# raphaelsulzer/dgnn

Measured on AMD Instinct MI355X. Metric: tetrahedra/sec (in/out classified), 1M-tet graph at 1/2/4/8 MI355X, higher is better.
Workload: dtype f32 (fp16x2-split products, 22-bit operands; `exact_f32` = bit-faithful fp32 products)

## Files before the change

### dgnn_amd/csrc/fused_ws.hip

```cpp
#include <stdlib.h>

#include "common.h"
#include "fused_common.h"

namespace {
using namespace fused;

typedef float f32x4_t __attribute__((ext_vector_type(4)));
#define H8(v) __builtin_bit_cast(f16x8, v)

constexpr int WS_C = 128;
constexpr int WS_TILE = 32;
constexpr int WS_NP = 8;
template <int CIN> struct WsC {
    static constexpr int NCH = CIN / 16;
    static constexpr int NV = NCH / 4;
    static constexpr int KH = CIN / 32;
    static constexpr int PP = CIN / 8;
    static constexpr int ROWB = 8 * CIN;
    static constexpr int SLOT = WS_TILE * ROWB;
    static constexpr int BP = NCH * 2 * 48 * 16;
};
template <int CIN, int RING> struct WsL {
    static constexpr int OFF_BP = RING * WsC<CIN>::SLOT;
    static constexpr int OFF_ROWF = OFF_BP + WsC<CIN>::BP;
    static constexpr int OFF_CST = OFF_ROWF + RING * WS_TILE * 4;
    static constexpr int OFF_SC = OFF_CST + 3 * WS_C * 4;
    static constexpr int OFF_DC = OFF_SC + 16 + 2 * RING * 4 + 16 + 16;
    static constexpr int OFF_PLOG = OFF_DC + (64 + 64 + 128 + 4) * 4;
    static constexpr int OFF_YS = OFF_PLOG + 2 * 4 * 32 * 8;
    static constexpr int OFF_CMAX = OFF_YS + 2 * 32 * 4;
    static constexpr int OFF_W0S = OFF_CMAX + 4 * 32 * 4;
    static constexpr int OFF_W0 = (OFF_W0S + 32 + 255) & ~255;
    static constexpr int OFF_YT = OFF_W0 + 4 * 4 * 2 * 64 * 16;
    static constexpr int SMEM = OFF_SC + 16 + 2 * RING * 4 + 16 + 16;
    static constexpr int SMEM_DEC = OFF_YT + 2 * 4 * 2 * 2 * 64 * 16;
    static_assert(SMEM_DEC <= 160 * 1024, "the LDS of one CU");
};

struct WsDec {
    const float* W0;
    const float* b0;
    const float* scale1;
    const float* shift1;
    const float* W3;
    const float* b3;
    float* logits;
};


__device__ __forceinline__ void st_nt16(float* p, f32x4_t v) { __builtin_nontemporal_store(v, reinterpret_cast<f32x4_t*>(p)); }
typedef uint32_t u32x2_t __attribute__((ext_vector_type(2)));
__device__ __forceinline__ float ub16_lo(uint32_t u) { return __builtin_fabsf(__builtin_bit_cast(float, u << 15)); }
__device__ __forceinline__ float ub16_hi(uint32_t u) { return __builtin_bit_cast(float, (u >> 16) << 15); }
__device__ __forceinline__ uint32_t ub16_enc(float v) {
    const uint32_t b = __builtin_bit_cast(uint32_t, v) & 0x7FFFFFFFu;
    return (b + 0x3FFFu + ((b >> 15) & 1u)) >> 15;
}
__device__ __forceinline__ uint32_t bits(float f) { return __builtin_bit_cast(uint32_t, f); }

constexpr int WS_KNOBS = 1 | (0 << 4);
template <int CIN, int RING, bool DEC, bool IO16 = false, bool LDC = false>
__global__ void __launch_bounds__(1024) k_sage_fused_ws(const int32_t* __restrict__ rowptr, const int32_t* __restrict__ src, const int32_t* __restrict__ eid,
                                                        int64_t n_dst, const float* __restrict__ x, const float* __restrict__ xdst, int64_t ldx_arg,
                                                        const float* __restrict__ ea, int64_t lde, const float* __restrict__ We, const float* __restrict__ be,
                                                        const float* __restrict__ Wj, const float* __restrict__ bj, const float* __restrict__ Wi,
                                                        const float* __restrict__ scale, const float* __restrict__ shift, int relu, float* __restrict__ out,
                                                        int64_t ldo, int64_t ntiles, int knobs, WsDec dec) {
    static_assert(CIN == 128 || (CIN == 64 && !DEC), "input widths of the shipped model's 128-wide layers");
    static_assert(!IO16 || !DEC, "the decoder-carrying launch of the bf16-storage chain stays with fused_bf16.hip");
    const int64_t ldx = LDC ? (int64_t)CIN : ldx_arg;
    const uint16_t* const x16 = reinterpret_cast<const uint16_t*>(x);
    const uint16_t* const xdst16 = reinterpret_cast<const uint16_t*>(xdst);
    uint16_t* const out16 = reinterpret_cast<uint16_t*>(out);
    typedef WsC<CIN> G;
    constexpr int NCH = G::NCH, NV = G::NV, KH = G::KH, PP = G::PP;
    extern __shared__ __attribute__((aligned(16))) char ws_smem[];
    const bool nt_store = (knobs & 1) != 0;
    typedef WsL<CIN, RING> L;
    char* const ring = ws_smem;
    char* const bpbuf = ws_smem + L::OFF_BP;
    float* const rowf = reinterpret_cast<float*>(ws_smem + L::OFF_ROWF);
    float* const cst = reinterpret_cast<float*>(ws_smem + L::OFF_CST);
    uint32_t* const scbuf = reinterpret_cast<uint32_t*>(ws_smem + L::OFF_SC);
    volatile uint32_t* const ready = reinterpret_cast<volatile uint32_t*>(ws_smem + L::OFF_SC + 16);
    volatile uint32_t* const done = ready + RING;
    volatile uint32_t* const ycnt = done + RING;
    volatile uint32_t* const yfree = ycnt + 2;
    volatile uint32_t* const lcnt = ycnt + 4;
    volatile uint32_t* const ccnt = ycnt + 6;
    float* const dcst = reinterpret_cast<float*>(ws_smem + L::OFF_DC);
    float* const plog = reinterpret_cast<float*>(ws_smem + L::OFF_PLOG);
    float* const ysc = reinterpret_cast<float*>(ws_smem + L::OFF_YS);
    uint32_t* const cmax = reinterpret_cast<uint32_t*>(ws_smem + L::OFF_CMAX);
    uint32_t* const w0max = reinterpret_cast<uint32_t*>(ws_smem + L::OFF_W0S);
    float* const w0inv = reinterpret_cast<float*>(ws_smem + L::OFF_W0S + 16);
    char* const w0buf = ws_smem + L::OFF_W0;
    char* const ytile = ws_smem + L::OFF_YT;
    typedef __attribute__((address_space(3))) volatile uint32_t lds_vu32;
    auto wait_for = [&](volatile uint32_t* ctr, uint32_t target) {
        asm volatile("" ::: "memory");
        lds_vu32* c3 = (lds_vu32*)ctr;
        while ((int32_t)(__builtin_amdgcn_readfirstlane((int)*c3) - (int)target) < 0) __builtin_amdgcn_s_sleep(1);
        asm volatile("" ::: "memory");
    };
    const int lane = lane_id(), w = wave_id_uniform();
    const int jcol = lane & 15, tq = lane >> 4;

    const int nwg = gridDim.x, xcd = blockIdx.x & 7, slot_ = blockIdx.x >> 3, wg_per_xcd = (nwg + 7 - xcd) >> 3;
    const int64_t per = (ntiles + 7) / 8, t_lo = xcd * per, t_hi = min(ntiles, t_lo + per);
    int64_t my_n = 0;
    if (t_lo + slot_ < t_hi) my_n = (t_hi - t_lo - slot_ + wg_per_xcd - 1) / wg_per_xcd;
    auto tile_of = [&](int64_t it) { return t_lo + slot_ + it * wg_per_xcd; };

    if (threadIdx.x == 0) scbuf[0] = 0u;
    if (threadIdx.x < 2 * RING + 8) ready[threadIdx.x] = 0u;
    if constexpr (DEC) {
        for (int n_ = threadIdx.x; n_ < 64; n_ += blockDim.x) {
            const float s1 = dec.scale1 ? dec.scale1[n_] : 1.f, h1 = dec.scale1 ? dec.shift1[n_] : 0.f;
            dcst[n_] = s1;
            dcst[64 + n_] = __fmaf_rn(dec.b0[n_], s1, h1);
            dcst[128 + n_] = dec.W3[n_];
            dcst[192 + n_] = dec.W3[64 + n_];
        }
        if (threadIdx.x < 2) dcst[256 + threadIdx.x] = dec.b3[threadIdx.x];
        if (threadIdx.x < 4 * WS_TILE) cmax[threadIdx.x] = 0u;
        if (threadIdx.x < 4) w0max[threadIdx.x] = 0u;
    }
    __syncthreads();
    if constexpr (DEC) {
#pragma unroll
        for (int hb = 0; hb < 4; ++hb) {
            uint32_t m0 = 0u;
            for (int e = threadIdx.x; e < 16 * WS_C; e += blockDim.x) m0 = umax(m0, absbits(dec.W0[hb * 16 * WS_C + e]));
            m0 = wave_umax(m0);
            if ((threadIdx.x & 63) == 0) atomicMax(&w0max[hb], m0);
        }
    }
    {
        uint32_t me = 0u;
        for (int e = threadIdx.x; e < CIN * FE; e += blockDim.x) me = umax(me, absbits(We[e]));
        for (int e = threadIdx.x; e < CIN; e += blockDim.x) me = umax(me, absbits(be[e]));
        me = wave_umax(me);
        if (lane == 0) atomicMax(&scbuf[0], me);
    }
    for (int c = threadIdx.x; c < WS_C; c += blockDim.x) {
        cst[c] = bj ? bj[c] : 0.f;
        cst[WS_C + c] = scale ? scale[c] : 1.f;
        cst[2 * WS_C + c] = scale ? shift[c] : 0.f;
    }
    __syncthreads();
    float sWe, inv_sWe;
    pow2_scales(scbuf[0], sWe, inv_sWe);
    constexpr bool LINE_OWN = !IO16 && NV == 2;
    auto chan = [](int j, int cb) { return LINE_OWN ? ((cb >> 2) * 64 + 4 * j + (cb & 3)) : NCH * j + cb; };
    for (int e = threadIdx.x; e < NCH * 48; e += blockDim.x) {
        const int cb = e / 48, gj = e - cb * 48, g = gj >> 4, j = gj & 15;
        const int c = chan(j, cb);
        uint32_t ph[4], pl[4];
#pragma unroll
        for (int d = 0; d < 4; ++d) {
            float v[2];
#pragma unroll
            for (int u = 0; u < 2; ++u) {
                const int k = 8 * g + 2 * d + u;
                v[u] = k < FE ? We[(int64_t)c * FE + k] : (k == FE ? be[c] : 0.f);
            }
            split2h(v[0] * sWe, v[1] * sWe, ph[d], pl[d]);
        }
        uint4* dst = reinterpret_cast<uint4*>(bpbuf + ((cb * 2) * 48 + gj) * 16);
        dst[0] = make_uint4(ph[0], ph[1], ph[2], ph[3]);
        dst[48] = make_uint4(pl[0], pl[1], pl[2], pl[3]);
    }

    auto stage_b = [&](uint32_t t, int hb, int b) {
        wait_for(ycnt + (t & 1), 8u * (t / 2 + 1));
        int ln = lane;
        asm volatile("" : "+v"(ln));
        const char* yt = ytile + ((t & 1) << 14) + ((b * 128 + ln) << 4);
        const char* wp = w0buf + ((hb * 512 + ln) << 4);
        const float inv = ysc[(t & 1) * WS_TILE + 16 * b + (ln & 15)] * w0inv[hb];
        f32x4_t hs = {0.f, 0.f, 0.f, 0.f};
#pragma unroll
        for (int s = 0; s < 4; ++s) {
            const f16x8 w0h = H8(*reinterpret_cast<const uint4*>(wp + (s << 11))), w0l = H8(*reinterpret_cast<const uint4*>(wp + (s << 11) + 1024));
            const f16x8 yh = H8(*reinterpret_cast<const uint4*>(yt + (s << 12))), yl = H8(*reinterpret_cast<const uint4*>(yt + (s << 12) + 1024));
            hs = __builtin_amdgcn_mfma_f32_16x16x32_f16(w0l, yh, hs, 0, 0, 0);
            hs = __builtin_amdgcn_mfma_f32_16x16x32_f16(w0h, yl, hs, 0, 0, 0);
            hs = __builtin_amdgcn_mfma_f32_16x16x32_f16(w0h, yh, hs, 0, 0, 0);
        }
        asm volatile("s_waitcnt lgkmcnt(0)" ::: "memory");
        if (lane == 0) atomicAdd(const_cast<uint32_t*>(yfree + (t & 1)), 1u);
#pragma unroll
        for (int i = 0; i < 4; ++i) hs[i] *= inv;
        const int u0 = 16 * hb + 4 * (ln >> 4);
        float l0 = 0.f, l1 = 0.f;
#pragma unroll
        for (int i = 0; i < 4; ++i) {
            const float hv = fmaxf(__fmaf_rn(hs[i], dcst[u0 + i], dcst[64 + u0 + i]), 0.f);
            l0 = __fmaf_rn(hv, dcst[128 + u0 + i], l0);
            l1 = __fmaf_rn(hv, dcst[192 + u0 + i], l1);
        }
        l0 = cross_row_sum(l0);
        l1 = cross_row_sum(l1);
        if (ln < 16) *reinterpret_cast<float2*>(plog + (((t & 1) * 4 + hb) * WS_TILE + 16 * b + ln) * 2) = make_float2(l0, l1);
        asm volatile("s_waitcnt lgkmcnt(0)" ::: "memory");
        if (lane == 0) atomicAdd(const_cast<uint32_t*>(lcnt + (t & 1)), 1u);
    };

    const int bsel = (knobs >> 4) & 3;
    auto b_on_consumers = [&](uint32_t t) { return bsel == 0 ? false : bsel == 1 ? (t & 1) == 0 : bsel == 2 ? (t & 3) != 3 : true; };

    if (w >= WS_NP) {
        const int cw = w - WS_NP;
        const int col = 16 * cw + jcol;
        uint32_t mw = 0u;
#pragma unroll
        for (int s = 0; s < 2 * KH; ++s) {
            const float* wr = (s < KH ? Wj : Wi) + (int64_t)col * CIN + 32 * (s % KH) + 8 * tq;
            const f32x4_t r0 = *reinterpret_cast<const f32x4_t*>(wr), r1 = *reinterpret_cast<const f32x4_t*>(wr + 4);
#pragma unroll
            for (int i = 0; i < 4; ++i) mw = umax(mw, umax(absbits(r0[i]), absbits(r1[i])));
        }
        float sW, inv_sW;
        pow2_scales(wave_umax(mw), sW, inv_sW);
        f16x8 wh[2 * KH], wl[2 * KH];
#pragma unroll
        for (int s = 0; s < 2 * KH; ++s) {
            const float* wr = (s < KH ? Wj : Wi) + (int64_t)col * CIN + 32 * (s % KH) + 8 * tq;
            const f32x4_t r0 = *reinterpret_cast<const f32x4_t*>(wr), r1 = *reinterpret_cast<const f32x4_t*>(wr + 4);
            uint32_t ph[4], pl[4];
            split2h(r0[0] * sW, r0[1] * sW, ph[0], pl[0]);
            split2h(r0[2] * sW, r0[3] * sW, ph[1], pl[1]);
            split2h(r1[0] * sW, r1[1] * sW, ph[2], pl[2]);
            split2h(r1[2] * sW, r1[3] * sW, ph[3], pl[3]);
            wh[s] = pack8h(ph);
            wl[s] = pack8h(pl);
        }
        if constexpr (DEC) {
#pragma unroll
            for (int u = 0; u < 2; ++u) {
                const int hb = 2 * (cw & 1) + u, ks = cw >> 1;
                float sW0, inv_sW0;
                pow2_scales(w0max[hb], sW0, inv_sW0);
                if (ks == 0 && lane == 0) w0inv[hb] = inv_sW0;
                const float* wr = dec.W0 + (int64_t)(16 * hb + jcol) * WS_C + 32 * ks + 8 * tq;
                const f32x4_t r0 = *reinterpret_cast<const f32x4_t*>(wr), r1 = *reinterpret_cast<const f32x4_t*>(wr + 4);
                uint32_t ph[4], pl[4];
                split2h(r0[0] * sW0, r0[1] * sW0, ph[0], pl[0]);
                split2h(r0[2] * sW0, r0[3] * sW0, ph[1], pl[1]);
                split2h(r1[0] * sW0, r1[1] * sW0, ph[2], pl[2]);
                split2h(r1[2] * sW0, r1[3] * sW0, ph[3], pl[3]);
                uint4* dst = reinterpret_cast<uint4*>(w0buf + (((hb * 4 + ks) * 128 + lane) << 4));
                dst[0] = make_uint4(ph[0], ph[1], ph[2], ph[3]);
                dst[64] = make_uint4(pl[0], pl[1], pl[2], pl[3]);
            }
        }
        __syncthreads();
        const int c0 = 16 * cw + 4 * tq;
        const int64_t n_it = my_n + (DEC ? 3 : 0);
        f32x4_t yp[2] = {{0.f, 0.f, 0.f, 0.f}, {0.f, 0.f, 0.f, 0.f}}, yn[2] = {yp[0], yp[1]};
        for (int64_t it = 1; it <= n_it; ++it) {
            if constexpr (DEC) {
                if (cw == 0 && it >= 4) {
                    const uint32_t t = (uint32_t)(it - 4);
                    wait_for(lcnt + (t & 1), 8u * (t / 2 + 1));
                    if (lane < WS_TILE) {
                        float s0 = dcst[256], s1 = dcst[257];
#pragma unroll
                        for (int q = 0; q < 4; ++q) {
                            const float* pq = plog + (((t & 1) * 4 + q) * WS_TILE + lane) * 2;
                            s0 += pq[0];
                            s1 += pq[1];
                        }
                        const int64_t cell = tile_of(t) * WS_TILE + lane;
                        if (cell < n_dst) *reinterpret_cast<float2*>(dec.logits + cell * 2) = make_float2(s0, s1);
                    }
                }
            }
            if (it >= 1 && it <= my_n) {
                const int sl = (int)((it - 1) % RING);
                wait_for(ready + sl, (uint32_t)(WS_NP * ((it - 1) / RING + 1)));
                f32x4_t acc[2] = {{0.f, 0.f, 0.f, 0.f}, {0.f, 0.f, 0.f, 0.f}};
                int key = jcol ^ tq;
                asm volatile("" : "+v"(key));
                uint32_t rbase[4];
#pragma unroll
                for (int m = 0; m < 4; ++m) {
                    rbase[m] = (uint32_t)(sl * G::SLOT + jcol * G::ROWB) + (uint32_t)(((4 * m) ^ key) << 4);
                    asm volatile("" : "+v"(rbase[m]));
                }
                f16x8 xh[2][2], xl[2][2];
                auto ld_step = [&](int s, int set) {
#pragma unroll
                    for (int b = 0; b < 2; ++b) {
                        const char* rp = ring + rbase[s & 3] + (16 * b * G::ROWB + ((s >> 2) << 8));
                        xh[set][b] = H8(*reinterpret_cast<const uint4*>(rp));
                        xl[set][b] = H8(*reinterpret_cast<const uint4*>(rp + 2 * PP * 16));
                    }
                };
                ld_step(0, 0);
#pragma unroll
                for (int s = 0; s < 2 * KH; ++s) {
                    const int set = s & 1;
                    if (s + 1 < 2 * KH) ld_step(s + 1, set ^ 1);
                    __builtin_amdgcn_sched_barrier(0);
#pragma unroll
                    for (int b = 0; b < 2; ++b) acc[b] = __builtin_amdgcn_mfma_f32_16x16x32_f16(wl[s], xh[set][b], acc[b], 0, 0, 0);
#pragma unroll
                    for (int b = 0; b < 2; ++b) acc[b] = __builtin_amdgcn_mfma_f32_16x16x32_f16(wh[s], xl[set][b], acc[b], 0, 0, 0);
#pragma unroll
                    for (int b = 0; b < 2; ++b) acc[b] = __builtin_amdgcn_mfma_f32_16x16x32_f16(wh[s], xh[set][b], acc[b], 0, 0, 0);
                    __builtin_amdgcn_sched_barrier(0);
                }
                float invr[2];
#pragma unroll
                for (int b = 0; b < 2; ++b) invr[b] = rowf[sl * WS_TILE + 16 * b + jcol] * inv_sW;
                asm volatile("s_waitcnt lgkmcnt(0)" ::: "memory");
                if (lane == 0) atomicAdd(const_cast<uint32_t*>(done + sl), 1u);
                const f32x4_t bb = *reinterpret_cast<const f32x4_t*>(cst + c0), sc = *reinterpret_cast<const f32x4_t*>(cst + WS_C + c0),
                              sh = *reinterpret_cast<const f32x4_t*>(cst + 2 * WS_C + c0);
                f32x4_t yv[2];
#pragma unroll
                for (int b = 0; b < 2; ++b) {
#pragma unroll
                    for (int i = 0; i < 4; ++i) {
                        float t_ = __fmaf_rn(acc[b][i], invr[b], bb[i]);
                        t_ = __fmaf_rn(t_, sc[i], sh[i]);
                        yv[b][i] = relu ? fmaxf(t_, 0.f) : t_;
                    }
                }
                if constexpr (!DEC) {
                    const int64_t cell0 = tile_of(it - 1) * WS_TILE;
#pragma unroll
                    for (int b = 0; b < 2; ++b) {
                        const int64_t cell = cell0 + 16 * b + jcol;
                        if (cell < n_dst) {
                            if constexpr (IO16) {
                                const u32x2_t pk = {ub16_enc(yv[b][0]) | (ub16_enc(yv[b][1]) << 16), ub16_enc(yv[b][2]) | (ub16_enc(yv[b][3]) << 16)};
                                if (nt_store) __builtin_nontemporal_store(pk, reinterpret_cast<u32x2_t*>(out16 + cell * ldo + c0));
                                else *reinterpret_cast<u32x2_t*>(out16 + cell * ldo + c0) = pk;
                            } else {
                                if (nt_store) st_nt16(out + cell * ldo + c0, yv[b]);
                                else *reinterpret_cast<f32x4_t*>(out + cell * ldo + c0) = yv[b];
                            }
                        }
                    }
                } else {
                    const uint32_t t = (uint32_t)(it - 1);
                    uint32_t* cm = cmax + (t & 3) * WS_TILE + jcol;
#pragma unroll
                    for (int b = 0; b < 2; ++b) {
                        const float my = fmaxf(fmaxf(fabsf(yv[b][0]), fabsf(yv[b][1])), fmaxf(fabsf(yv[b][2]), fabsf(yv[b][3])));
                        atomicMax(cm + 16 * b, ((t / 4 + 1) << 8) | (bits(my) >> 23));
                    }
                    asm volatile("s_waitcnt lgkmcnt(0)" ::: "memory");
                    if (lane == 0) atomicAdd(const_cast<uint32_t*>(ccnt + (t & 1)), 1u);
                    yn[0] = yv[0], yn[1] = yv[1];
                }
            }
            if constexpr (DEC) {
                if (it >= 2 && it <= my_n + 1) {
                    const uint32_t t = (uint32_t)(it - 2);
                    wait_for(ccnt + (t & 1), 8u * (t / 2 + 1));
                    wait_for(yfree + (t & 1), 8u * (t / 2));
                    int ln = lane;
                    asm volatile("" : "+v"(ln));
                    const uint32_t* cm = cmax + (t & 3) * WS_TILE + (ln & 15);
                    char* yt = ytile + ((t & 1) << 14) + ((cw >> 1) << 12) + (((ln & 15) + 16 * (2 * (cw & 1) + (ln >> 5))) << 4) + (((ln >> 4) & 1) << 3);
#pragma unroll
                    for (int b = 0; b < 2; ++b) {
                        float sY, inv_sY;
                        pow2_scales((cm[16 * b] & 255u) << 23, sY, inv_sY);
                        uint32_t ph[2], pl[2];
                        split2h(yp[b][0] * sY, yp[b][1] * sY, ph[0], pl[0]);
                        split2h(yp[b][2] * sY, yp[b][3] * sY, ph[1], pl[1]);
                        *reinterpret_cast<uint2*>(yt + (b << 11)) = make_uint2(ph[0], ph[1]);
                        *reinterpret_cast<uint2*>(yt + (b << 11) + 1024) = make_uint2(pl[0], pl[1]);
                        if (cw == 0 && ln < 16) ysc[(t & 1) * WS_TILE + 16 * b + ln] = inv_sY;
                    }
                    asm volatile("s_waitcnt lgkmcnt(0)" ::: "memory");
                    if (lane == 0) atomicAdd(const_cast<uint32_t*>(ycnt + (t & 1)), 1u);
                }
                yp[0] = yn[0], yp[1] = yn[1];
                if (it >= 3 && it <= my_n + 2 && b_on_consumers((uint32_t)(it - 3))) stage_b((uint32_t)(it - 3), cw & 3, cw >> 2);
            }
        }
        return;
    }

    __syncthreads();
    const int p = w;
    const int P0 = NCH * jcol;
    const int Q0 = 4 * jcol;
    const int n_my = (int)my_n;
    const int it_short = (n_my > 0 && tile_of(n_my - 1) == ntiles - 1) ? n_my - 1 : -1;
    const int nv_short = (int)max((int64_t)0, min((int64_t)4, n_dst - ((ntiles - 1) * WS_TILE + 4 * p)));
    auto nv_of = [&](int it) { return it == it_short ? nv_short : 4; };
    auto load_rp = [&](int it, int& vb) {
        if (it < n_my) {
            const int64_t i0 = tile_of(it) * WS_TILE + 4 * p;
            const int nv = nv_of(it);
            vb = nv > 0 ? rowptr[i0 + (lane < nv ? lane : nv)] : 0;
        }
    };
    typedef int32_t i32x4a_t __attribute__((ext_vector_type(4), aligned(4)));
    constexpr bool IDX_LANE = !DEC;
    auto load_idx = [&](int it, int vb, bool& reg, int (&vs)[4], int& veid) {
        reg = false;
        if (it < n_my) {
            const int nv = nv_of(it);
            if (nv > 0) {
                const int b0 = __builtin_amdgcn_readfirstlane(vb);
                reg = __all(vb == b0 + 4 * (lane < nv ? lane : nv)) != 0;
                if (reg) {
                    if constexpr (IDX_LANE) {
                        const i32x4a_t s4 = *reinterpret_cast<const i32x4a_t*>(src + b0 + 4 * (tq < nv ? tq : nv - 1));
                        vs[0] = s4[0], vs[1] = s4[1], vs[2] = s4[2], vs[3] = s4[3];
                        const int k_e = b0 + (jcol < 4 * nv ? jcol : 4 * nv - 1);
                        veid = eid ? eid[k_e] : k_e;
                    } else {
                        const int k_me = b0 + (lane < 4 * nv ? lane : 4 * nv - 1);
                        vs[0] = src[k_me];
                        veid = eid ? eid[k_me] : k_me;
                    }
                }
            }
        }
    };
    int vb1 = 0, vb2 = 0, vs1[4] = {0, 0, 0, 0}, veid1 = 0;
    bool reg1 = false;
    load_rp(0, vb1);
    load_rp(1, vb2);
    load_idx(0, vb1, reg1, vs1, veid1);

    for (int it = 0; it < n_my + (DEC ? 3 : 0); ++it) {
        int nv = 0, sl = 0, tl = 0, vs[4] = {0, 0, 0, 0}, veid = 0;
        bool regular = false;
        f32x4_t xo[NV], q0, q1, rr[4][NV];
        uint32_t xo16[NCH / 2], rr16[4][NCH / 2];
        int64_t cell = 0;
        auto own_row = [&]() {
            if constexpr (IO16) {
                const uint16_t* rp0 = xdst16 + cell * ldx + P0;
                if constexpr (NCH == 8) {
                    const uint4 u = *reinterpret_cast<const uint4*>(rp0);
                    xo16[0] = u.x, xo16[1] = u.y, xo16[2] = u.z, xo16[3] = u.w;
                } else {
                    const uint2 u = *reinterpret_cast<const uint2*>(rp0);
                    xo16[0] = u.x, xo16[1] = u.y;
                }
            } else {
                const float* rp0 = xdst + cell * ldx + (LINE_OWN ? Q0 : P0);
#pragma unroll
                for (int v = 0; v < NV; ++v) xo[v] = *reinterpret_cast<const f32x4_t*>(rp0 + (LINE_OWN ? 64 : 4) * v);
            }
        };
        auto neighbour_rows = [&]() {
            auto src_of = [&](int r) {
                if constexpr (IDX_LANE) return vs[r];
                else return __shfl(vs[0], tl * 4 + r);
            };
            auto eid_of = [&]() {
                if constexpr (IDX_LANE) return veid;
                else return __shfl(veid, jcol);
            };
            const float* er = ea + (int64_t)eid_of() * lde;
            q0 = *reinterpret_cast<const f32x4_t*>(er + 8 * (tq < 2 ? tq : 2));
            q1 = *reinterpret_cast<const f32x4_t*>(er + 8 * (tq < 1 ? tq : 1) + 4);
#pragma unroll
            for (int r = 0; r < 4; ++r) {
                if constexpr (IO16) {
                    const uint16_t* rp = x16 + (int64_t)src_of(r) * ldx + P0;
                    if constexpr (NCH == 8) {
                        const uint4 u = *reinterpret_cast<const uint4*>(rp);
                        rr16[r][0] = u.x, rr16[r][1] = u.y, rr16[r][2] = u.z, rr16[r][3] = u.w;
                    } else {
                        const uint2 u = *reinterpret_cast<const uint2*>(rp);
                        rr16[r][0] = u.x, rr16[r][1] = u.y;
                    }
                } else {
                    const float* rp = x + (int64_t)src_of(r) * ldx + (LINE_OWN ? Q0 : P0);
#pragma unroll
                    for (int v = 0; v < NV; ++v) rr[r][v] = *reinterpret_cast<const f32x4_t*>(rp + (LINE_OWN ? 64 : 4) * v);
                }
            }
        };
        if (it < n_my) {
            const int64_t i0 = tile_of(it) * WS_TILE + 4 * p;
            sl = it % RING;
            nv = nv_of(it);
            regular = reg1;
#pragma unroll
            for (int r = 0; r < 4; ++r) vs[r] = vs1[r];
            veid = veid1;
            vb1 = vb2;
            load_idx(it + 1, vb1, reg1, vs1, veid1);
            load_rp(it + 2, vb2);
            tl = tq < nv ? tq : nv - 1;
            cell = i0 + tl;
        }
        if constexpr (DEC) {
            if (it < n_my && nv > 0) {
                own_row();
                if (regular) neighbour_rows();
            }
            if (it >= 3 && !b_on_consumers((uint32_t)(it - 3))) stage_b((uint32_t)(it - 3), p & 3, p >> 2);
        }
        if (it < n_my) {
            if (nv > 0) {
                if constexpr (!DEC) own_row();
                float aout[NCH], xv[NCH];
#pragma unroll
                for (int v = 0; v < NV; ++v) {
#pragma unroll
                    for (int i = 0; i < 4; ++i) {
                        if constexpr (IO16) xv[4 * v + i] = (i & 1) ? ub16_hi(xo16[2 * v + (i >> 1)]) : ub16_lo(xo16[2 * v + (i >> 1)]);
                        else xv[4 * v + i] = xo[v][i];
                    }
                }
                if (regular) {
                    if constexpr (!DEC) neighbour_rows();
                    float av[8];
#pragma unroll
                    for (int i = 0; i < 4; ++i) {
                        av[i] = tq < 3 ? q0[i] : 0.f;
                        av[4 + i] = tq < 2 ? q1[i] : 0.f;
                    }
                    if (tq == 2) av[4] = 1.0f;
                    float mf = 0.f;
#pragma unroll
                    for (int i = 0; i < 8; i += 2) mf = fmaxf(fmaxf(mf, fabsf(av[i])), fabsf(av[i + 1]));
                    float sA, inv_sA;
                    pow2_scales(cross_row_umax(bits(mf)), sA, inv_sA);
                    uint32_t ph[4], pl[4];
#pragma unroll
                    for (int d = 0; d < 4; ++d) split2h(av[2 * d] * sA, av[2 * d + 1] * sA, ph[d], pl[d]);
                    float inv_e[4];
#pragma unroll
                    for (int r = 0; r < 4; ++r) inv_e[r] = __shfl(inv_sA, 4 * tq + r);
                    const f16x8 ah = pack8h(ph), al = pack8h(pl);
#pragma unroll
                    for (int c4 = 0; c4 < NCH; c4 += 2) {
                        f16x8 bh[2], bl[2];
                        f32x4_t d[2];
#pragma unroll
                        for (int u = 0; u < 2; ++u) {
                            const char* bp = bpbuf + (((c4 + u) * 2) * 48 + (tq < 3 ? tq : 0) * 16 + jcol) * 16;
                            bh[u] = H8(*reinterpret_cast<const uint4*>(bp));
                            bl[u] = H8(*reinterpret_cast<const uint4*>(bp + 768));
                            d[u] = f32x4_t{0.f, 0.f, 0.f, 0.f};
                        }
#pragma unroll
                        for (int u = 0; u < 2; ++u) d[u] = __builtin_amdgcn_mfma_f32_16x16x32_f16(al, bh[u], d[u], 0, 0, 0);
#pragma unroll
                        for (int u = 0; u < 2; ++u) d[u] = __builtin_amdgcn_mfma_f32_16x16x32_f16(ah, bl[u], d[u], 0, 0, 0);
#pragma unroll
                        for (int u = 0; u < 2; ++u) d[u] = __builtin_amdgcn_mfma_f32_16x16x32_f16(ah, bh[u], d[u], 0, 0, 0);
#pragma unroll
                        for (int u = 0; u < 2; ++u) {
                            const int c8 = c4 + u;
#pragma unroll
                            for (int r = 0; r < 4; ++r) d[u][r] *= inv_e[r];
                            auto nb_ = [&](int r) {
                                if constexpr (IO16) return (c8 & 1) ? ub16_hi(rr16[r][c8 >> 1]) : ub16_lo(rr16[r][c8 >> 1]);
                                else return rr[r][c8 >> 2][c8 & 3];
                            };
                            float a = __fmul_rn(nb_(0), d[u][0]);
#pragma unroll
                            for (int r = 1; r < 4; ++r) a = __fmaf_rn(nb_(r), d[u][r], a);
                            aout[c8] = a * (0.25f * inv_sWe);
                        }
                    }
                } else {
#pragma unroll
                    for (int cb = 0; cb < NCH; ++cb) aout[cb] = 0.f;
                    if (tq < nv) {
                        const int b = rowptr[cell], e_end = rowptr[cell + 1];
                        for (int k = b; k < e_end; ++k) {
                            const int s_ = src[k];
                            const float* ar = ea + (int64_t)(eid ? eid[k] : k) * lde;
#pragma unroll 1
                            for (int cb = 0; cb < NCH; ++cb) {
                                const int c = chan(jcol, cb);
                                float pf = be[c];
                                for (int f = 0; f < FE; ++f) pf = __fmaf_rn(We[(int64_t)c * FE + f], ar[f], pf);
                                const float xs_ = IO16 ? __builtin_bit_cast(float, (uint32_t)x16[(int64_t)s_ * ldx + c] << 15) : x[(int64_t)s_ * ldx + c];
                                aout[cb] = __fadd_rn(aout[cb], __fmul_rn(xs_, pf));
                            }
                        }
                        const float cnt = (float)max(e_end - b, 1);
#pragma unroll
                        for (int cb = 0; cb < NCH; ++cb) aout[cb] = __fdiv_rn(aout[cb], cnt);
                    }
                }
                float ma = 0.f;
#pragma unroll
                for (int i = 0; i < NCH; i += 2) {
                    ma = fmaxf(fmaxf(ma, fabsf(aout[i])), fabsf(aout[i + 1]));
                    ma = fmaxf(fmaxf(ma, fabsf(xv[i])), fabsf(xv[i + 1]));
                }
                float s_, inv_;
                pow2_scales(row16_umax(bits(ma)), s_, inv_);
                const int T = 4 * p + tq;
                wait_for(done + sl, (uint32_t)(8 * (it / RING)));
                if (jcol == 0) rowf[sl * WS_TILE + T] = inv_;
                uint32_t ah_[NCH / 2], al_[NCH / 2], xh_[NCH / 2], xl_[NCH / 2];
#pragma unroll
                for (int d = 0; d < NCH / 2; ++d) {
                    split2h(aout[2 * d] * s_, aout[2 * d + 1] * s_, ah_[d], al_[d]);
                    split2h(xv[2 * d] * s_, xv[2 * d + 1] * s_, xh_[d], xl_[d]);
                }
                char* rowp = ring + sl * G::SLOT + T * G::ROWB;
                const int key = T & 15;
                if constexpr (LINE_OWN) {
                    const int half = (jcol & 1) << 3;
#pragma unroll
                    for (int qd = 0; qd < 2; ++qd) {
                        const int pc = 8 * qd + (jcol >> 1);
                        *reinterpret_cast<uint2*>(rowp + ((pc ^ key) << 4) + half) = make_uint2(ah_[2 * qd], ah_[2 * qd + 1]);
                        *reinterpret_cast<uint2*>(rowp + (((PP + pc) ^ key) << 4) + half) = make_uint2(xh_[2 * qd], xh_[2 * qd + 1]);
                        *reinterpret_cast<uint2*>(rowp + (((2 * PP + pc) ^ key) << 4) + half) = make_uint2(al_[2 * qd], al_[2 * qd + 1]);
                        *reinterpret_cast<uint2*>(rowp + (((3 * PP + pc) ^ key) << 4) + half) = make_uint2(xl_[2 * qd], xl_[2 * qd + 1]);
                    }
                } else if constexpr (NCH == 8) {
                    *reinterpret_cast<uint4*>(rowp + ((jcol ^ key) << 4)) = make_uint4(ah_[0], ah_[1], ah_[2], ah_[3]);
                    *reinterpret_cast<uint4*>(rowp + (((PP + jcol) ^ key) << 4)) = make_uint4(xh_[0], xh_[1], xh_[2], xh_[3]);
                    *reinterpret_cast<uint4*>(rowp + (((2 * PP + jcol) ^ key) << 4)) = make_uint4(al_[0], al_[1], al_[2], al_[3]);
                    *reinterpret_cast<uint4*>(rowp + (((3 * PP + jcol) ^ key) << 4)) = make_uint4(xl_[0], xl_[1], xl_[2], xl_[3]);
                } else {
                    const int pc = jcol >> 1, half = (jcol & 1) << 3;
                    *reinterpret_cast<uint2*>(rowp + ((pc ^ key) << 4) + half) = make_uint2(ah_[0], ah_[1]);
                    *reinterpret_cast<uint2*>(rowp + (((PP + pc) ^ key) << 4) + half) = make_uint2(xh_[0], xh_[1]);
                    *reinterpret_cast<uint2*>(rowp + (((2 * PP + pc) ^ key) << 4) + half) = make_uint2(al_[0], al_[1]);
                    *reinterpret_cast<uint2*>(rowp + (((3 * PP + pc) ^ key) << 4) + half) = make_uint2(xl_[0], xl_[1]);
                }
            } else {
                wait_for(done + sl, (uint32_t)(8 * (it / RING)));
            }
            asm volatile("s_waitcnt lgkmcnt(0)" ::: "memory");
            if (lane == 0) atomicAdd(const_cast<uint32_t*>(ready + sl), 1u);
        }
    }
}

}

int dgnn_ws_enabled() {
    static const int v = getenv("DGNN_WS") ? atoi(getenv("DGNN_WS")) : 1;
    return v;
}

extern "C" int dgnn_wave_specialised_enabled(void) { return dgnn_ws_enabled() != 0 ? 1 : 0; }

int dgnn_sage_layer_fused_ws_try(const LayerCall& c, const DecoderTail& t) {
    const bool dec = t.W0 != nullptr;
    if ((c.c_in != WS_C && !(c.c_in == 64 && !dec)) || c.c_out != WS_C || c.lde != FE || c.ldx % 4 != 0 || (!dec && c.ldo % 4 != 0) ||
        ((((uintptr_t)c.x_src | (uintptr_t)c.x_dst | (uintptr_t)c.edge_attr | (uintptr_t)(dec ? nullptr : c.out) | (uintptr_t)c.Wj | (uintptr_t)c.Wi |
           (uintptr_t)t.W0) % 16) != 0) ||
        (dec && ((uintptr_t)t.logits % 8) != 0))
        return DGNN_E_UNSUPPORTED;
    static const int ws64 = getenv("DGNN_WS_64") ? atoi(getenv("DGNN_WS_64")) : 1;
    if (c.c_in == 64 && !ws64) return DGNN_E_UNSUPPORTED;
    const int64_t ntiles = dgnn_cdiv(c.n_dst, WS_TILE);
    int grid = (int)(ntiles < DGNN_NUM_CU ? ntiles : DGNN_NUM_CU);
    if (grid < 1) grid = 1;
    const WsDec d{t.W0, t.b0, t.scale1, t.shift1, t.W3, t.b3, t.logits};
    const bool ldc = c.ldx == c.c_in;
#define DGNN_WS_GO(C_, D_, L_)                                                                                                                              \
    do {                                                                                                                                                    \
        static bool attr_[DGNN_MAX_DEVICES] = {};                                                                                                           \
        const size_t sm_ = D_ ? WsL<C_, 2>::SMEM_DEC : WsL<C_, 2>::SMEM;                                                                                    \
        dgnn_allow_dynamic_lds(reinterpret_cast<const void*>(&k_sage_fused_ws<C_, 2, D_, false, L_>), sm_, attr_);                                          \
        hipLaunchKernelGGL((k_sage_fused_ws<C_, 2, D_, false, L_>), dim3(grid), dim3(1024), sm_, c.stream, c.rowptr, c.src, c.eid, c.n_dst, c.x_src,        \
                           c.x_dst, c.ldx, c.edge_attr, c.lde, c.We, c.be, c.Wj, c.bj, c.Wi, c.scale, c.shift, c.relu, c.out, c.ldo, ntiles, WS_KNOBS, d);  \
    } while (0)
#define DGNN_WS_GO2(C_, D_)                \
    do {                                   \
        if (ldc) DGNN_WS_GO(C_, D_, true); \
        else DGNN_WS_GO(C_, D_, false);    \
    } while (0)
    if (c.c_in == 64) DGNN_WS_GO2(64, false);
    else if (dec) DGNN_WS_GO2(128, true);
    else DGNN_WS_GO2(128, false);
#undef DGNN_WS_GO2
#undef DGNN_WS_GO
    return dgnn_check_launch(dec ? "sage_layer_fused_decoder_fwd(wave-specialised)" : "sage_layer_fused_fwd(wave-specialised)");
}

int dgnn_sage_layer_fused_ws16_try(const LayerCall16& c) {
    static const int on = getenv("DGNN_WS_16") ? atoi(getenv("DGNN_WS_16")) : 1;
    const int nch = c.c_in / 16;
    if (!on || !dgnn_ws_enabled() || (c.c_in != 128 && c.c_in != 64) || c.c_out != WS_C || !c.relu || c.lde != FE || c.ldx % nch != 0 || c.ldo % 4 != 0 ||
        ((((uintptr_t)c.x_src | (uintptr_t)c.x_dst) % (2 * nch)) != 0) || ((uintptr_t)c.out % 8) != 0 ||
        ((((uintptr_t)c.edge_attr | (uintptr_t)c.Wj | (uintptr_t)c.Wi) % 16) != 0))
        return DGNN_E_UNSUPPORTED;
    const int64_t ntiles = dgnn_cdiv(c.n_dst, WS_TILE);
    int grid = (int)(ntiles < DGNN_NUM_CU ? ntiles : DGNN_NUM_CU);
    if (grid < 1) grid = 1;
    const WsDec d{};
    const float* xs = static_cast<const float*>(c.x_src);
    const float* xd = static_cast<const float*>(c.x_dst);
    float* o = reinterpret_cast<float*>(c.out);
    const bool ldc = c.ldx == c.c_in;
#define DGNN_WS_GO16(C_, R_, L_)                                                                                                                            \
    do {                                                                                                                                                    \
        static bool attr_[DGNN_MAX_DEVICES] = {};                                                                                                           \
        const size_t sm_ = WsL<C_, R_>::SMEM;                                                                                                               \
        dgnn_allow_dynamic_lds(reinterpret_cast<const void*>(&k_sage_fused_ws<C_, R_, false, true, L_>), sm_, attr_);                                       \
        hipLaunchKernelGGL((k_sage_fused_ws<C_, R_, false, true, L_>), dim3(grid), dim3(1024), sm_, c.stream, c.rowptr, c.src, c.eid, c.n_dst, xs, xd,      \
                           c.ldx, c.edge_attr, c.lde, c.We, c.be, c.Wj, c.bj, c.Wi, c.scale, c.shift, c.relu, o, c.ldo, ntiles, WS_KNOBS, d);               \
    } while (0)
    if (c.c_in == 64) {
        if (ldc) DGNN_WS_GO16(64, 4, true);
        else DGNN_WS_GO16(64, 4, false);
    } else {
        if (ldc) DGNN_WS_GO16(128, 2, true);
        else DGNN_WS_GO16(128, 2, false);
    }
#undef DGNN_WS_GO16
    return dgnn_check_launch("sage_layer_fused_fwd_bf16(wave-specialised)");
}
```

Measured before the change: 752.0 million.

## Pack edge-filter split products into two MFMAs instead of three

Repacks the fp16 hi/lo split edge-filter weights and the per-lane edge attributes so that the 62 needed cross terms (hi*hi, hi*lo, lo*hi over 21 k values) fit densely into two 16x16x32 MFMA operands rather than three. Previously the three-MFMA scheme used padded k groups of 48 slots. A constexpr slot map with static_asserts checks that each term appears exactly once. The intent is to cut the MFMA count in the message/aggregation inner loop by a third. The cost is a larger B-pack in LDS (64 rows instead of 48) and extra per-lane selects to build the A operand.

```diff
diff --git a/dgnn_amd/csrc/filter_pack.h b/dgnn_amd/csrc/filter_pack.h
--- /dev/null
+++ b/dgnn_amd/csrc/filter_pack.h
@@ -0,0 +1,92 @@
+#pragma once
+
+namespace filter_pack {
+
+constexpr int FE = 20;
+constexpr int NK = FE + 1;
+constexpr int NTERMS = 3 * NK - 1;
+
+enum Part : signed char { NONE = 0, HI = 1, LO = 2 };
+struct Slot {
+    signed char a, b;
+    signed char k;
+};
+constexpr int M2 = 0, M1 = 1;
+
+#define FP_ROW8(a, b, k0)                                                                                                              \
+    {Slot{a, b, k0}, Slot{a, b, k0 + 1}, Slot{a, b, k0 + 2}, Slot{a, b, k0 + 3}, Slot{a, b, k0 + 4}, Slot{a, b, k0 + 5}, Slot{a, b, k0 + 6}, \
+     Slot{a, b, k0 + 7}}
+#define FP_W(a, b, k0) Slot{a, b, k0}, Slot{a, b, k0 + 1}
+#define FP_WC(b) Slot{HI, b, FE}, Slot{NONE, NONE, -1}
+constexpr Slot MAP[2][4][8] = {
+    {{FP_W(LO, HI, 0), FP_W(LO, HI, 2), FP_W(HI, LO, 2), FP_W(HI, LO, 0)},
+     {FP_W(HI, LO, 12), FP_W(HI, LO, 14), FP_W(LO, HI, 12), FP_W(LO, HI, 14)},
+     {FP_W(LO, HI, 16), FP_W(LO, HI, 18), FP_W(HI, LO, 18), FP_WC(LO)},
+     {FP_W(LO, HI, 4), FP_W(LO, HI, 6), FP_W(LO, HI, 8), FP_W(LO, HI, 10)}},
+    {FP_ROW8(HI, HI, 0), FP_ROW8(HI, HI, 8),
+     {FP_W(HI, HI, 16), FP_W(HI, HI, 18), FP_WC(HI), FP_W(HI, LO, 16)},
+     FP_ROW8(HI, LO, 4)},
+};
+#undef FP_W
+#undef FP_WC
+#undef FP_ROW8
+
+constexpr int count_term(int a, int b, int k) {
+    int n = 0;
+    for (int m = 0; m < 2; ++m)
+        for (int g = 0; g < 4; ++g)
+            for (int s = 0; s < 8; ++s) n += MAP[m][g][s].a == a && MAP[m][g][s].b == b && MAP[m][g][s].k == k;
+    return n;
+}
+constexpr bool terms_once() {
+    int used = 0;
+    for (int k = 0; k < NK; ++k) {
+        if (count_term(HI, HI, k) != 1 || count_term(HI, LO, k) != 1) return false;
+        if (count_term(LO, HI, k) != (k < FE ? 1 : 0) || count_term(LO, LO, k) != 0) return false;
+    }
+    for (int m = 0; m < 2; ++m)
+        for (int g = 0; g < 4; ++g)
+            for (int s = 0; s < 8; ++s) {
+                const Slot t = MAP[m][g][s];
+                if (t.k >= 0) {
+                    if (t.k >= NK || t.a == NONE || t.b == NONE) return false;
+                    ++used;
+                } else if (t.a != NONE || t.b != NONE) {
+                    return false;
+                }
+            }
+    return used == NTERMS;
+}
+constexpr bool words_whole() {
+    for (int m = 0; m < 2; ++m)
+        for (int g = 0; g < 4; ++g)
+            for (int d = 0; d < 4; ++d) {
+                const Slot e = MAP[m][g][2 * d], o = MAP[m][g][2 * d + 1];
+                if (e.k < 0 || (e.k & 1)) return false;
+                if (e.k == FE ? o.k != -1 : (o.k != e.k + 1 || o.a != e.a || o.b != e.b)) return false;
+            }
+    return true;
+}
+constexpr int LANE_K[4][8] = {{0, 1, 2, 3, 4, 5, 6, 7}, {8, 9, 10, 11, 12, 13, 14, 15}, {16, 17, 18, 19, FE, -1, 16, 17}, {4, 5, 6, 7, 8, 9, 10, 11}};
+constexpr bool m1_is_hi() {
+    for (int g = 0; g < 4; ++g)
+        for (int s = 0; s < 8; ++s)
+            if (MAP[M1][g][s].k != LANE_K[g][s] || (MAP[M1][g][s].k >= 0 && MAP[M1][g][s].a != HI)) return false;
+    return true;
+}
+constexpr bool m2_is_own() {
+    for (int g = 0; g < 4; ++g)
+        for (int d = 0; d < 4; ++d) {
+            bool found = false;
+            for (int i = 0; i < 4; ++i) found = found || LANE_K[g][2 * i] == MAP[M2][g][2 * d].k;
+            if (!found) return false;
+        }
+    return true;
+}
+constexpr bool a_word(int m, int g, int d, int a, int k) { return MAP[m][g][2 * d].a == a && MAP[m][g][2 * d].k == k; }
+static_assert(terms_once(), "62 terms, each once");
+static_assert(words_whole(), "whole words of one part");
+static_assert(m1_is_hi(), "M1 = the hi words of the lane's eight values");
+static_assert(m2_is_own(), "M2 = words of the lane's eight values");
+
+}
diff --git a/dgnn_amd/csrc/fused_ws.hip b/dgnn_amd/csrc/fused_ws.hip
--- a/dgnn_amd/csrc/fused_ws.hip
+++ b/dgnn_amd/csrc/fused_ws.hip
@@ -1,6 +1,7 @@
 #include <stdlib.h>
 
 #include "common.h"
+#include "filter_pack.h"
 #include "fused_common.h"
 
 namespace {
@@ -19,7 +20,7 @@
     static constexpr int PP = CIN / 8;
     static constexpr int ROWB = 8 * CIN;
     static constexpr int SLOT = WS_TILE * ROWB;
-    static constexpr int BP = NCH * 2 * 48 * 16;
+    static constexpr int BP = NCH * 2 * 64 * 16;
 };
 template <int CIN, int RING> struct WsL {
     static constexpr int OFF_BP = RING * WsC<CIN>::SLOT;
@@ -154,23 +155,26 @@
     pow2_scales(scbuf[0], sWe, inv_sWe);
     constexpr bool LINE_OWN = !IO16 && NV == 2;
     auto chan = [](int j, int cb) { return LINE_OWN ? ((cb >> 2) * 64 + 4 * j + (cb & 3)) : NCH * j + cb; };
-    for (int e = threadIdx.x; e < NCH * 48; e += blockDim.x) {
-        const int cb = e / 48, gj = e - cb * 48, g = gj >> 4, j = gj & 15;
+    for (int e = threadIdx.x; e < NCH * 16; e += blockDim.x) {
+        const int cb = e >> 4, j = e & 15;
         const int c = chan(j, cb);
-        uint32_t ph[4], pl[4];
-#pragma unroll
-        for (int d = 0; d < 4; ++d) {
-            float v[2];
-#pragma unroll
-            for (int u = 0; u < 2; ++u) {
-                const int k = 8 * g + 2 * d + u;
-                v[u] = k < FE ? We[(int64_t)c * FE + k] : (k == FE ? be[c] : 0.f);
-            }
-            split2h(v[0] * sWe, v[1] * sWe, ph[d], pl[d]);
-        }
-        uint4* dst = reinterpret_cast<uint4*>(bpbuf + ((cb * 2) * 48 + gj) * 16);
-        dst[0] = make_uint4(ph[0], ph[1], ph[2], ph[3]);
-        dst[48] = make_uint4(pl[0], pl[1], pl[2], pl[3]);
+        uint32_t wh[11], wl[11];
+#pragma unroll
+        for (int i = 0; i < 10; ++i) split2h(We[(int64_t)c * FE + 2 * i] * sWe, We[(int64_t)c * FE + 2 * i + 1] * sWe, wh[i], wl[i]);
+        split2h(be[c] * sWe, 0.f, wh[10], wl[10]);
+#pragma unroll
+        for (int m = 0; m < 2; ++m) {
+#pragma unroll
+            for (int g = 0; g < 4; ++g) {
+                uint32_t wd[4];
+#pragma unroll
+                for (int d = 0; d < 4; ++d) {
+                    const filter_pack::Slot t = filter_pack::MAP[m][g][2 * d];
+                    wd[d] = t.k < 0 ? 0u : (t.b == filter_pack::HI ? wh[t.k >> 1] : wl[t.k >> 1]);
+                }
+                *reinterpret_cast<uint4*>(bpbuf + (((cb * 2 + m) * 64 + g * 16 + j) << 4)) = make_uint4(wd[0], wd[1], wd[2], wd[3]);
+            }
+        }
     }
 
     auto stage_b = [&](uint32_t t, int hb, int b) {
@@ -466,8 +470,8 @@
                 else return __shfl(veid, jcol);
             };
             const float* er = ea + (int64_t)eid_of() * lde;
-            q0 = *reinterpret_cast<const f32x4_t*>(er + 8 * (tq < 2 ? tq : 2));
-            q1 = *reinterpret_cast<const f32x4_t*>(er + 8 * (tq < 1 ? tq : 1) + 4);
+            q0 = *reinterpret_cast<const f32x4_t*>(er + (tq < 3 ? 8 * tq : 4));
+            q1 = *reinterpret_cast<const f32x4_t*>(er + (tq < 2 ? 8 * tq + 4 : (tq == 2 ? 4 : 8)));
 #pragma unroll
             for (int r = 0; r < 4; ++r) {
                 if constexpr (IO16) {
@@ -521,13 +525,24 @@
                 }
                 if (regular) {
                     if constexpr (!DEC) neighbour_rows();
+                    using filter_pack::HI;
+                    using filter_pack::LO;
+                    static_assert(filter_pack::a_word(filter_pack::M2, 0, 0, LO, 0) && filter_pack::a_word(filter_pack::M2, 0, 1, LO, 2) &&
+                                      filter_pack::a_word(filter_pack::M2, 0, 2, HI, 2) && filter_pack::a_word(filter_pack::M2, 0, 3, HI, 0) &&
+                                      filter_pack::a_word(filter_pack::M2, 1, 0, HI, 12) && filter_pack::a_word(filter_pack::M2, 1, 1, HI, 14) &&
+                                      filter_pack::a_word(filter_pack::M2, 1, 2, LO, 12) && filter_pack::a_word(filter_pack::M2, 1, 3, LO, 14) &&
+                                      filter_pack::a_word(filter_pack::M2, 2, 0, LO, 16) && filter_pack::a_word(filter_pack::M2, 2, 1, LO, 18) &&
+                                      filter_pack::a_word(filter_pack::M2, 2, 2, HI, 18) && filter_pack::a_word(filter_pack::M2, 2, 3, HI, 20) &&
+                                      filter_pack::a_word(filter_pack::M2, 3, 0, LO, 4) && filter_pack::a_word(filter_pack::M2, 3, 3, LO, 10) &&
+                                      filter_pack::LANE_K[2][4] == FE && filter_pack::LANE_K[2][6] == 16 && filter_pack::LANE_K[3][0] == 4,
+                                  "the loads and selects here follow the map");
                     float av[8];
 #pragma unroll
-                    for (int i = 0; i < 4; ++i) {
-                        av[i] = tq < 3 ? q0[i] : 0.f;
-                        av[4 + i] = tq < 2 ? q1[i] : 0.f;
-                    }
-                    if (tq == 2) av[4] = 1.0f;
+                    for (int i = 0; i < 4; ++i) av[i] = q0[i];
+                    av[4] = tq == 2 ? 1.0f : q1[0];
+                    av[5] = tq == 2 ? 0.f : q1[1];
+                    av[6] = tq == 2 ? q0[0] : q1[2];
+                    av[7] = tq == 2 ? q0[1] : q1[3];
                     float mf = 0.f;
 #pragma unroll
                     for (int i = 0; i < 8; i += 2) mf = fmaxf(fmaxf(mf, fabsf(av[i])), fabsf(av[i + 1]));
@@ -539,24 +554,23 @@
                     float inv_e[4];
 #pragma unroll
                     for (int r = 0; r < 4; ++r) inv_e[r] = __shfl(inv_sA, 4 * tq + r);
-                    const f16x8 ah = pack8h(ph), al = pack8h(pl);
+                    const uint32_t p2[4] = {tq == 1 ? ph[2] : pl[0], tq == 1 ? ph[3] : pl[1], (tq & 1) ? pl[2] : ph[1], (tq & 1) ? pl[3] : (tq == 0 ? ph[0] : ph[2])};
+                    const f16x8 a1 = pack8h(ph), a2 = pack8h(p2);
 #pragma unroll
                     for (int c4 = 0; c4 < NCH; c4 += 2) {
-                        f16x8 bh[2], bl[2];
+                        f16x8 b2[2], b1[2];
                         f32x4_t d[2];
 #pragma unroll
                         for (int u = 0; u < 2; ++u) {
-                            const char* bp = bpbuf + (((c4 + u) * 2) * 48 + (tq < 3 ? tq : 0) * 16 + jcol) * 16;
-                            bh[u] = H8(*reinterpret_cast<const uint4*>(bp));
-                            bl[u] = H8(*reinterpret_cast<const uint4*>(bp + 768));
+                            const char* bp = bpbuf + ((((c4 + u) * 2) * 64 + lane) << 4);
+                            b2[u] = H8(*reinterpret_cast<const uint4*>(bp));
+                            b1[u] = H8(*reinterpret_cast<const uint4*>(bp + 1024));
                             d[u] = f32x4_t{0.f, 0.f, 0.f, 0.f};
                         }
 #pragma unroll
-                        for (int u = 0; u < 2; ++u) d[u] = __builtin_amdgcn_mfma_f32_16x16x32_f16(al, bh[u], d[u], 0, 0, 0);
-#pragma unroll
-                        for (int u = 0; u < 2; ++u) d[u] = __builtin_amdgcn_mfma_f32_16x16x32_f16(ah, bl[u], d[u], 0, 0, 0);
-#pragma unroll
-                        for (int u = 0; u < 2; ++u) d[u] = __builtin_amdgcn_mfma_f32_16x16x32_f16(ah, bh[u], d[u], 0, 0, 0);
+                        for (int u = 0; u < 2; ++u) d[u] = __builtin_amdgcn_mfma_f32_16x16x32_f16(a2, b2[u], d[u], 0, 0, 0);
+#pragma unroll
+                        for (int u = 0; u < 2; ++u) d[u] = __builtin_amdgcn_mfma_f32_16x16x32_f16(a1, b1[u], d[u], 0, 0, 0);
 #pragma unroll
                         for (int u = 0; u < 2; ++u) {
                             const int c8 = c4 + u;
```

Result: faster. 770.1 million, median of 6 (+2.4%).
